# adjo0043/Mathematical-Modeling-Of-Infectious-Diseases-V1

Measured on AMD Instinct MI355X. Metric: ODE-solve+likelihood evals/sec (SEPAIHRD 4-age, 400d), higher is better.
Workload: dtype f64

## Files before the change

mathematical-modeling-of-infectious-diseases-v1_amd/csrc/phase_pass.py:

```python
#!/usr/bin/env python3
import argparse, os, re, subprocess, sys, tempfile

LLVM = "/opt/rocm/lib/llvm/bin"
MCPU = "gfx950"
E64_OK = re.compile(r"^\s+(v_fmac_f64_e32|v_mov_b32_e32|v_mov_b64_e32|v_add_u32_e32|v_sub_u32_e32|v_subrev_u32_e32|v_mul_f32_e32|v_add_f32_e32|"
                    r"v_cvt_f32_f64_e32|v_cvt_f64_f32_e32|v_cvt_f64_i32_e32|v_rcp_f64_e32|v_log_f32_e32|v_exp_f32_e32|v_and_b32_e32|v_or_b32_e32|"
                    r"v_lshlrev_b32_e32|v_max_i32_e32|v_min_i32_e32)\b")


def assemble_sizes(path):
    tmp = tempfile.mkdtemp(prefix="pp_")
    obj = os.path.join(tmp, "a.o")
    subprocess.run([LLVM + "/clang", "-x", "assembler", "-target", "amdgcn-amd-amdhsa", "-mcpu=" + MCPU, "-c", path, "-o", obj], check=True,
                   stdout=subprocess.DEVNULL, stderr=subprocess.DEVNULL)
    dis = subprocess.run([LLVM + "/llvm-objdump", "-d", obj], check=True, capture_output=True, text=True).stdout
    out, cur = {}, None
    for line in dis.splitlines():
        m = re.match(r"^[0-9a-f]+ <(\S+)>:", line)
        if m:
            cur = out.setdefault(m.group(1), [])
            continue
        m = re.match(r"^\s+(\S+).*//\s*([0-9A-Fa-f]+):\s+((?:[0-9A-Fa-f]{8}\s*)+)", line)
        if m and cur is not None:
            cur.append((int(m.group(2), 16), 4 * len(m.group(3).split()), m.group(1)))
# ... 72 lines not shown
        m = re.match(r"^(\w+):\s*(;.*)?$", l)
        if m and m.group(1) in sizes:
            func = m.group(1); funcs[func] = []
            continue
        if l.startswith("\t.end_amdhsa_kernel") or l.strip().startswith(".Lfunc_end"):
            func = None
        if func is not None and is_instruction(l):
            funcs[func].append(i)
    n_re = n_nop = n_runs = n_fixed = 0
    edits = {}
    inserts = {}
    for name, idxs in funcs.items():
        if not any(w in name for w in wanted):
            continue
        ins = sizes[name]
        if len(ins) != len(idxs):
            print(f"skip {name[:70]}: {len(ins)} disassembled vs {len(idxs)} listed instructions", file=sys.stderr)
            continue
        guarded = protected_spans(lines, idxs)
        start = 0
        shift = 0
        for k in range(len(ins) + 1):
            end_block = k == len(ins) or ins[k][2].startswith(("s_cbranch", "s_branch", "s_endpgm", "s_setpc"))
            if not end_block:
                continue
            blk = list(range(start, min(k + 1, len(ins))))
            start = k + 1
            if len(blk) < args.min_block:
                continue
            j = 0
            last_touch = -1
            while j < len(blk):
                a = blk[j]
                if ins[a][1] != 8:
                    j += 1
                    continue
                r = j
                while r < len(blk) and ins[blk[r]][1] == 8:
                    r += 1
                run_len = r - j
                if run_len >= args.min_run:
                    n_runs += 1
                    if (ins[a][0] + shift) % 8 == 4:
                        fixed = False
                        for b in range(j - 1, max(j - 1 - args.look_back, last_touch), -1):
                            li = idxs[blk[b]]
                            if blk[b] in guarded:
                                continue
                            if ins[blk[b]][1] == 4 and li not in edits and E64_OK.match(lines[li]) and "0x" not in lines[li] and "dpp" not in lines[li] and "sdwa" not in lines[li]:
                                edits[li] = lines[li].replace("_e32", "_e64", 1)
                                shift += 4; n_re += 1; fixed = True; last_touch = b
                                break
                        if not fixed and run_len >= args.nop_run and a not in guarded:
                            inserts[idxs[a]] = "\ts_nop 0"
                            shift += 4; n_nop += 1; fixed = True; last_touch = j
                        n_fixed += fixed
                j = r
    out = []
    for i, l in enumerate(lines):
        if i in inserts:
            out.append(inserts[i])
        out.append(edits.get(i, l))
    open(args.dst, "w").write("\n".join(out))
    try:
        after = assemble_sizes(args.dst)
    except subprocess.CalledProcessError:
        print("phase_pass: the rewritten assembly does not assemble", file=sys.stderr)
        sys.exit(1)
    if args.body_residue >= 0:
        out_lines = open(args.dst).read().split("\n")
        inserts_at = {}
        for name, ins in after.items():
            if "sepaihrd_eval_quad_kernel" not in name or not ins:
                continue
            blocks, start = [], 0
            for k in range(len(ins) + 1):
                if k == len(ins) or ins[k][2].startswith(("s_cbranch", "s_branch", "s_endpgm", "s_setpc")):
                    blocks.append(ins[start:min(k + 1, len(ins))]); start = k + 1
            bodies = [b for b in blocks if len(b) >= args.min_block and sum(1 for _, _, m in b if "f64" in m or "dpp" in m) * 2 > len(b)]
            if not bodies:
                continue
            body = min(bodies, key=len)
            delta = (args.body_residue - body[0][0]) % 64
            delta -= delta % 8
            if delta:
                inserts_at[name] = delta // 4
        if inserts_at:
            padded = []
            for l in out_lines:
                padded.append(l)
                m = re.match(r"^(\w+):\s*(;.*)?$", l)
                if m and m.group(1) in inserts_at:
                    padded.extend(["\ts_nop 0"] * inserts_at[m.group(1)])
            open(args.dst, "w").write("\n".join(padded))
            try:
                after = assemble_sizes(args.dst)
            except subprocess.CalledProcessError:
                print("phase_pass: the padded assembly does not assemble", file=sys.stderr)
                sys.exit(1)
            print(f"body residue {args.body_residue}: entry pads {sorted(set(inserts_at.values()))} s_nop in {len(inserts_at)} kernels")
    runs_before, off_before = off_phase_runs(sizes, wanted, args.min_run, args.min_block)
    runs_after, off_after = off_phase_runs(after, wanted, args.min_run, args.min_block)
    print(f"runs of >= {args.min_run} wide encodings: {n_runs}; off phase and fixed: {n_fixed} ({n_re} re-encoded, {n_nop} s_nop); "
          f"off-phase runs by the assembled addresses: {off_before} of {runs_before} before, {off_after} of {runs_after} after")
    if off_after > off_before:
        print("phase_pass: the rewritten assembly has MORE off-phase runs than its input", file=sys.stderr)
        sys.exit(1)


if __name__ == "__main__":
    main()
```

mathematical-modeling-of-infectious-diseases-v1_amd/csrc/sepaihrd_capi.cpp:

```cpp
#include "sepaihrd_hip.h"

#include <hip/hip_runtime.h>
#include <dlfcn.h>

#include <algorithm>
#include <cmath>
#include <cstdio>
#include <cstdlib>
#include <cstring>
#include <limits>
#include <string>
#include <vector>

#include "sepaihrd_device.h"
#include "sepaihrd_fd_device.h"
#include "sepaihrd_host_util.h"
#include "sepaihrd_mh_backend.h"
#include "sepaihrd_predictive_device.h"
#include "sepaihrd_segments.h"
#include "sepaihrd_stoch_sepaihrd_device.h"

using namespace sepaihrd;

enum EnsSlot {
// ... 263 lines not shown
    ctx->precision = pb->precision;
    ctx->n = n; ctx->T = T; ctx->P = P;
    ctx->host_N.assign(pb->N, pb->N + n);
    if (const char* mb = std::getenv("SEPAIHRD_WORKSPACE_MB")) {
        const long v = std::atol(mb);
        if (v > 0) ctx->ws_budget_bytes = (size_t)v << 20;
    }

    const int lpc = lanes_per_chain(n);
    const int ns = SS_SCHEDULE0 + nb + nk;

    std::vector<int32_t> src_scalar(ns, -1);
    std::vector<double> base_scalar(ns, 0.0);
    base_scalar[SS_BETA] = pb->beta; base_scalar[SS_THETA] = pb->theta; base_scalar[SS_SIGMA] = pb->sigma;
    base_scalar[SS_GAMMA_P] = pb->gamma_p; base_scalar[SS_GAMMA_A] = pb->gamma_A;
    base_scalar[SS_GAMMA_I] = pb->gamma_I; base_scalar[SS_GAMMA_H] = pb->gamma_H;
    base_scalar[SS_GAMMA_ICU] = pb->gamma_ICU;
    for (int i = 0; i < 8; ++i) base_scalar[SS_E0_MULT + i] = pb->multipliers[i];
    base_scalar[SS_RUNUP_DAYS] = pb->runup_days; base_scalar[SS_SEED_EXPOSED] = pb->seed_exposed;
    for (int k = 0; k < nb; ++k) base_scalar[SS_SCHEDULE0 + k] = pb->beta_values[k];
    for (int k = 0; k < nk; ++k) base_scalar[SS_SCHEDULE0 + nb + k] = pb->kappa_values[k];

    std::vector<int32_t> src_vec((size_t)VF_COUNT * lpc, -1);
    std::vector<double> base_vec((size_t)VF_COUNT * lpc, 0.0);
    const double* vec_base_ptr[VF_COUNT] = {pb->a, pb->h_infec, pb->p, pb->h, pb->icu, pb->d_H, pb->d_ICU,
                                            pb->d_community};
    for (int f = 0; f < VF_COUNT; ++f)
        for (int i = 0; i < n; ++i) base_vec[(size_t)f * lpc + i] = vec_base_ptr[f] ? vec_base_ptr[f][i] : 0.0;

    int kappa_calibrated = 0;
    for (int p = 0; p < P; ++p) {
        const int f = pb->param_field[p], idx = pb->param_index[p];
        auto bad = [&](const char* what) {
            set_err(err, errlen, std::string("param ") + std::to_string(p) + ": " + what);
            delete ctx;
            return static_cast<sepaihrd_ctx*>(nullptr);
        };
        if (f == SEPAIHRD_F_NONE) continue;
        if (f >= SEPAIHRD_F_BETA && f <= SEPAIHRD_F_SEED_EXPOSED) {
            src_scalar[f] = p;
        } else if (f == SEPAIHRD_F_BETA_VALUE) {
            if (idx < 0 || idx >= nb) return bad("beta index out of range");
            src_scalar[SS_SCHEDULE0 + idx] = p;
        } else if (f == SEPAIHRD_F_KAPPA_VALUE) {
            if (idx < 1 || idx >= nk) return bad("kappa index out of range (index 0 is the fixed baseline)");
            src_scalar[SS_SCHEDULE0 + nb + idx] = p;
            kappa_calibrated = 1;
        } else if (f >= SEPAIHRD_F_A && f <= SEPAIHRD_F_D_COMMUNITY) {
            if (idx < 0 || idx >= n) return bad("age index out of range");
            src_vec[(size_t)(f - SEPAIHRD_F_A) * lpc + idx] = p;
        } else {
            return bad("unknown field code");
        }
    }

    std::vector<double> Npad(lpc, 0.0), fracpad(lpc, 0.0), Mrow((size_t)lpc * lpc, 0.0),
        init((size_t)NUM_COMP * lpc, 0.0);
    double total_pop = 0.0;
    for (int i = 0; i < n; ++i) { Npad[i] = pb->N[i]; total_pop += pb->N[i]; }
    if (total_pop > 0.0)
        for (int i = 0; i < n; ++i) fracpad[i] = pb->N[i] / total_pop;
    for (int i = 0; i < n; ++i)
        for (int j = 0; j < n; ++j) Mrow[(size_t)i * lpc + j] = pb->M[(size_t)j * n + i];
    for (int c = 0; c < NUM_COMP; ++c)
        for (int i = 0; i < n; ++i) init[(size_t)c * lpc + i] = pb->initial_state[(size_t)c * n + i];

    int runup_offset = 0;
    for (int i = 0; i < T; ++i)
        if (pb->times[i] >= 0.0) { runup_offset = i; break; }
    const int num_obs_points = T - runup_offset;
    const int n_obs = pb->n_obs;
    const double qnan = std::numeric_limits<double>::quiet_NaN();
    std::vector<double> grid((size_t)T * lpc * 4, qnan);
    const double* obs_ptr[3] = {pb->obs_H, pb->obs_ICU, pb->obs_D};
    for (int k = 0; k < T; ++k)
        for (int i = 0; i < lpc; ++i) {
            double* rec = &grid[((size_t)k * lpc + i) * 4];
            const int r = k - runup_offset;
            if (i < n && r >= 0 && r < n_obs)
                for (int s = 0; s < 3; ++s) rec[s] = obs_ptr[s][(size_t)r * n + i];
            rec[3] = pb->times[k + 1 < T ? k + 1 : T - 1];
        }

    std::vector<double> mends;
    for (int k = 0; k < nb; ++k) mends.push_back(pb->beta_end_times[k]);
    for (int k = 0; k < nk; ++k) mends.push_back(pb->kappa_end_times[k]);
    std::sort(mends.begin(), mends.end());
    mends.erase(std::unique(mends.begin(), mends.end()), mends.end());
    const int nm = (int)mends.size();
    std::vector<int32_t> seg_ib(nm + 1, 0), seg_ik(nm + 1, 0);
    for (int j = 0; j <= nm; ++j) {
        const double trep = j < nm ? mends[j] : std::numeric_limits<double>::infinity();
        int cb = 0, ckk = 0;
        for (int k = 0; k < nb; ++k) cb += (trep > pb->beta_end_times[k]) ? 1 : 0;
        for (int k = 0; k < nk; ++k) ckk += (trep > pb->kappa_end_times[k]) ? 1 : 0;
        seg_ib[j] = nb > 0 ? std::min(cb, nb - 1) : 0;
        seg_ik[j] = std::min(ckk, nk - 1);
    }
    if (nm & 1) mends.push_back(std::numeric_limits<double>::infinity());

    double max_gap = 0.0;
    for (int i = 1; i < T; ++i) max_gap = std::max(max_gap, pb->times[i] - pb->times[i - 1]);

    ctx->lower.assign(P, 0.0); ctx->upper.assign(P, 0.0); ctx->has_bounds.assign(P, 0);
    std::vector<int32_t> hb(P, 0);
    for (int p = 0; p < P; ++p) {
        const bool has = pb->has_bounds ? pb->has_bounds[p] != 0 : (pb->lower && pb->upper);
        ctx->has_bounds[p] = has ? 1 : 0;
        hb[p] = has ? 1 : 0;
        if (has) { ctx->lower[p] = pb->lower[p]; ctx->upper[p] = pb->upper[p]; }
    }

    DevProblem& d = ctx->dp;
    d.n = n; d.lpc = lpc; d.T = T; d.n_obs = n_obs; d.runup_offset = runup_offset; d.nb = nb; d.nk = nk;
    d.P = P; d.ns = ns;
    d.constraint_mode = pb->constraint_mode == SEPAIHRD_CONSTRAINT_REFLECT ? 1 : 0;
    d.kappa_calibrated = kappa_calibrated;
    d.max_attempts = pb->max_attempts > 0 ? pb->max_attempts : 1000000;
    d.obs_rows_match = (num_obs_points == n_obs) ? 1 : 0;
    d.abs_tol = pb->abs_err; d.rel_tol = pb->rel_err; d.dt_hint = pb->dt_hint; d.max_gap = max_gap;

    bool ok = true;
    d.times = upload(ctx->allocs, std::vector<double>(pb->times, pb->times + T), ok);
    d.grid = upload(ctx->allocs, grid, ok);
    d.lower = upload(ctx->allocs, ctx->lower, ok);
    d.upper = upload(ctx->allocs, ctx->upper, ok);
    d.has_bounds = upload(ctx->allocs, hb, ok);
    d.src_scalar = upload(ctx->allocs, src_scalar, ok);
    d.base_scalar = upload(ctx->allocs, base_scalar, ok);
    d.src_vec = upload(ctx->allocs, src_vec, ok);
    d.base_vec = upload(ctx->allocs, base_vec, ok);
    d.N = upload(ctx->allocs, Npad, ok);
    d.age_fraction = upload(ctx->allocs, fracpad, ok);
    d.Mrow = upload(ctx->allocs, Mrow, ok);
    d.init_state = upload(ctx->allocs, init, ok);
    d.beta_ends = upload(ctx->allocs, std::vector<double>(pb->beta_end_times, pb->beta_end_times + nb), ok);
    d.kappa_ends = upload(ctx->allocs, std::vector<double>(pb->kappa_end_times, pb->kappa_end_times + nk), ok);
    d.nm = nm; d.nm_pad = (int)mends.size();
    d.mends = upload(ctx->allocs, mends, ok);
    d.seg_ib = upload(ctx->allocs, seg_ib, ok);
    d.seg_ik = upload(ctx->allocs, seg_ik, ok);
    if (!ok) {
        set_err(err, errlen, "device allocation / upload failed");
        sepaihrd_destroy(ctx);
        return nullptr;
    }
    if (eval_lds_bytes(d) + LOG_TABLE_LDS_BYTES > 64 * 1024) {
        set_err(err, errlen, "n_params too large for the LDS staging buffer");
        sepaihrd_destroy(ctx);
        return nullptr;
    }
    return ctx;
}

void sepaihrd_destroy(sepaihrd_ctx* ctx) {
    if (!ctx) return;
    (void)hipSetDevice(ctx->device);
    delete ctx;
}

const char* sepaihrd_last_error(const sepaihrd_ctx* ctx) { return ctx ? ctx->last_error.c_str() : "ctx is NULL"; }

int sepaihrd_set_constraint_mode(sepaihrd_ctx* ctx, int mode) {
    if (!ctx || (mode != SEPAIHRD_CONSTRAINT_CLAMP && mode != SEPAIHRD_CONSTRAINT_REFLECT))
        return SEPAIHRD_E_INVALID_ARG;
    ctx->dp.constraint_mode = mode;
    return SEPAIHRD_OK;
}

int sepaihrd_set_arith(sepaihrd_ctx* ctx, int arith) {
    if (!ctx || (arith != SEPAIHRD_ARITH_STRICT && arith != SEPAIHRD_ARITH_FMA)) return SEPAIHRD_E_INVALID_ARG;
    ctx->arith = arith;
    return SEPAIHRD_OK;
}

int sepaihrd_set_precision(sepaihrd_ctx* ctx, int precision) {
    if (!ctx || (precision != SEPAIHRD_PRECISION_F64 && precision != SEPAIHRD_PRECISION_F32)) return SEPAIHRD_E_INVALID_ARG;
    if (precision == SEPAIHRD_PRECISION_F32 && ctx->dp.lpc < 4) {
        ctx->last_error = "the fp32-state arm is built for 3 to 16 age classes";
        return SEPAIHRD_E_UNSUPPORTED;
    }
    if (precision == SEPAIHRD_PRECISION_F32 && ctx->solver == SEPAIHRD_SOLVER_FEHLBERG78) {
        ctx->last_error = "the fp32-state arm is built for Dopri5 and Cash-Karp only";
        return SEPAIHRD_E_UNSUPPORTED;
    }
    ctx->precision = precision;
    return SEPAIHRD_OK;
}

int sepaihrd_reserve(sepaihrd_ctx* ctx, int max_B) {
    if (!ctx || max_B < 0) return SEPAIHRD_E_INVALID_ARG;
    HIP_TRY(hipSetDevice(ctx->device), ctx, return SEPAIHRD_E_HIP);
    return ensure_workspace(ctx, chunk_chains(ctx, (size_t)max_B));
}

int sepaihrd_eval_batch_device(sepaihrd_ctx* ctx, const double* d_theta, int B, double* d_loglik,
                               int32_t* d_status, int32_t* d_n_accept, int32_t* d_n_reject,
                               double* d_ll_parts, double* d_traj, void* stream) {
    if (!ctx) return SEPAIHRD_E_INVALID_ARG;
    if (B < 0 || (B > 0 && (!d_theta || !d_loglik))) {
        ctx->last_error = "eval_batch_device: NULL theta/loglik or negative B";
        return SEPAIHRD_E_INVALID_ARG;
    }
    if (B == 0) return SEPAIHRD_OK;
    const int needs = needs_workspace(ctx, B, 0);
    if (needs < 0) { ctx->last_error = "unsupported lanes-per-chain"; return SEPAIHRD_E_UNSUPPORTED; }
    const bool split = needs != 0;
// ... 1910 lines not shown
```

mathematical-modeling-of-infectious-diseases-v1_amd/csrc/sepaihrd_device.h:

```cpp
#pragma once
#include <stdint.h>

namespace sepaihrd {

constexpr int NUM_COMP = 11;
constexpr int NUM_POP_COMP = 9;
constexpr int WAVE = 64;

enum ScalarSlot {
    SS_BETA = 0, SS_THETA, SS_SIGMA, SS_GAMMA_P, SS_GAMMA_A, SS_GAMMA_I, SS_GAMMA_H, SS_GAMMA_ICU,
    SS_E0_MULT, SS_P0_MULT, SS_A0_MULT, SS_I0_MULT, SS_H0_MULT, SS_ICU0_MULT, SS_R0_MULT, SS_D0_MULT,
    SS_RUNUP_DAYS, SS_SEED_EXPOSED,
    SS_SCHEDULE0
};
enum VecField { VF_A = 0, VF_H_INFEC, VF_P, VF_H, VF_ICU, VF_D_H, VF_D_ICU, VF_D_COMM, VF_COUNT };

struct DevProblem {
    int32_t n, lpc, T, n_obs, runup_offset, nb, nk, P, ns;
    int32_t constraint_mode, kappa_calibrated, max_attempts, obs_rows_match;
    int32_t init_mode;
    int32_t form;
    double abs_tol, rel_tol, dt_hint, max_gap;
    const double* times;
    const double* grid;
    const double* lower;
    const double* upper;
    const int32_t* has_bounds;
    const int32_t* src_scalar;
    const double* base_scalar;
    const int32_t* src_vec;
    const double* base_vec;
    const double* N;
    const double* age_fraction;
    const double* Mrow;
    const double* init_state;
    const double* beta_ends;
    const double* kappa_ends;
    int32_t nm, nm_pad;
    const double* mends;
    const int32_t* seg_ib;
    const int32_t* seg_ik;
};

struct EvalOutputs {
    double* loglik;
    int32_t* status;
    int32_t* n_accept;
    int32_t* n_reject;
    double* ll_parts;
    double* traj;
    double* cum;
    double* rows;
    int32_t* wstatus;
    void* ev_after_integrator;
    int32_t force_split;
};
inline size_t workspace_cum_doubles(const DevProblem& pb, size_t chains) { return (size_t)pb.T * 3 * chains * pb.lpc; }
constexpr size_t CUM_ROW_DOUBLES = 3 * WAVE;
#if defined(__HIPCC__)
__host__ __device__
#endif
inline size_t cum_index(int T, size_t column, int day, int comp) {
    return ((column / WAVE) * (size_t)T + (size_t)day) * CUM_ROW_DOUBLES + (size_t)comp * WAVE + (column % WAVE);
}
inline size_t workspace_rows_doubles(const DevProblem& pb, size_t chains) { return (size_t)pb.T * 3 * chains; }

constexpr int LL_FORM_INLINE = 0, LL_FORM_SEPARATE_PASS = 1, LL_FORM_CONSUMER_WAVES = 2;
struct LaunchInfo {
    int vgprs, sgprs, lds_static, lds_dynamic, scratch, max_blocks_per_cu;
    int lanes_per_chain;
    int likelihood_form;
    const char* name;
};

int launch_eval_strict(const DevProblem& pb, int solver, const double* d_theta, int B,
                       const EvalOutputs& out, void* stream);
int launch_eval_fma(const DevProblem& pb, int solver, const double* d_theta, int B,
                    const EvalOutputs& out, void* stream);
int launch_eval_scenario_strict(const DevProblem& pb, int solver, const double* d_theta, int B, const EvalOutputs& out, void* stream,
                                const double* d_kappa_mult, int stride);
int launch_eval_scenario_fma(const DevProblem& pb, int solver, const double* d_theta, int B, const EvalOutputs& out, void* stream,
                             const double* d_kappa_mult, int stride);
int launch_needs_workspace_strict(const DevProblem& pb, int solver, int B, int force_split);
int launch_needs_workspace_fma(const DevProblem& pb, int solver, int B, int force_split);
int launch_eval_f32(const DevProblem& pb, int solver, const double* d_theta, int B, const EvalOutputs& out, void* stream);
int kernel_info_f32(const DevProblem& pb, int solver, LaunchInfo* info);
int kernel_info_strict(const DevProblem& pb, int solver, int batch, LaunchInfo* info);
int kernel_info_fma(const DevProblem& pb, int solver, int batch, LaunchInfo* info);
int phase_pass_applied_strict();
int phase_pass_applied_fma();
int poisson_log_values(const double* d_x, int n, double* d_out, void* stream);

constexpr int ENSEMBLE_MAX_SAMPLES = 16384;
struct EnsembleArgs {
    int S, S_pad;
    int lpc, n, T, Tp;
    int runup_offset;
    int n_probs;
    size_t cum_stride;
    const double* cum;
    const int32_t* wstatus;
    const double* traj;
    double total_pop;
    double* vals;
    const double* probs;
    double* q_out;
    double* sero_out;
    int32_t* n_valid;
    double* rt_out;
    int rt_segment0;
    const DevProblem* pb;
    const double* theta;
    double* metrics_out;
    double* sort_scratch;
    size_t sort_scratch_doubles;
};
int launch_ensemble_summaries(const EnsembleArgs& a, void* stream);
struct ScenarioArgs {
    int K, S, S_pad, W;
    int n_probs;
    const double* probs;
    const double* metrics;
    const int32_t* wstatus;
    size_t status_stride;
    double* vals;
// ... 103 lines not shown
```

mathematical-modeling-of-infectious-diseases-v1_amd/csrc/sepaihrd_lane_split.inc:

```

constexpr int QUAD_LANES = 16;
constexpr int QUAD_CPW = WAVE / QUAD_LANES;
constexpr int QUAD_SLOTS = 3;

template <int CTRL>
__device__ __forceinline__ double quad_rot(double v) { return dpp_move<CTRL>(v); }
constexpr int QROT_LEFT = 0x93;
constexpr int QROT_NEXT = 0x39;

#ifndef SEPAIHRD_STRICT_STAGE_PADS
#define SEPAIHRD_STRICT_STAGE_PADS 0
#endif
#define SEP_STAGE_PAD(i, v) do { if ((SEPAIHRD_STRICT_STAGE_PADS >> (i)) & 1) asm volatile("s_nop 0" : "+v"(v)); } while (0)
#ifndef SEPAIHRD_STRICT_HEAD_PADS_CK
#define SEPAIHRD_STRICT_HEAD_PADS_CK 0
#endif
#ifndef SEPAIHRD_STRICT_STAGE_PADS_CK
#define SEPAIHRD_STRICT_STAGE_PADS_CK 0
#endif
#define SEP_STAGE_PAD_CK(i, v) do { if ((SEPAIHRD_STRICT_STAGE_PADS_CK >> (i)) & 1) asm volatile("s_nop 0" : "+v"(v)); } while (0)
#define SEP_PHASE_PAD(n) do { if ((n) >= 1) asm volatile("s_nop 0"); if ((n) >= 2) asm volatile("s_nop 0"); if ((n) >= 3) asm volatile("s_nop 0"); } while (0)
using lanemask = unsigned long long;
__device__ __forceinline__ lanemask lanes_where(bool p) { return __builtin_amdgcn_ballot_w64(p); }
__device__ __forceinline__ bool lane_of(lanemask m) { return __builtin_amdgcn_inverse_ballot_w64(m); }
__device__ __forceinline__ double min_plain(double a, double b) {
    double r;
    asm("v_min_f64 %0, %1, %2" : "=v"(r) : "v"(a), "v"(b));
    return r;
}

#if SEPAIHRD_ARITH_FMA
struct QuadModel {
    double theta_inf, m[4];
    double cO1, cL1;
    double cO0, cX0, cL0;
    double a1, a2, a3, a4, a5;
};

__device__ __forceinline__ void rhs_quad(const QuadModel& q, const double (&x)[QUAD_SLOTS], double (&dx)[QUAD_SLOTS],
                                         double beta_eff) {
    const double Lx1 = quad_rot<QROT_LEFT>(x[1]);
    const double Nx1 = quad_rot<QROT_NEXT>(x[1]), Nx0 = quad_rot<QROT_NEXT>(x[0]);
    const double pressure = fma(q.theta_inf, x[1], Lx1 + x[0]);
    double lambda = 0.0;
    fmac_row_bcast<2, 0xf, true>(lambda, pressure, q.m[0]);
    fmac_row_bcast<6, 0xf, false>(lambda, pressure, q.m[1]);
    fmac_row_bcast<10, 0xf, false>(lambda, pressure, q.m[2]);
    fmac_row_bcast<14, 0xf, false>(lambda, pressure, q.m[3]);
    lambda *= beta_eff;
    const double lambda_val = (0.0 < lambda) ? lambda : 0.0;
    const double W = lambda_val * x[0];
    dx[1] = fma(q.cO1, x[1], fma(q.cL1, Lx1, W));
    dx[0] = fma(q.cO0, x[0], fma(q.cX0, x[1], fma(q.cL0, Lx1, -W)));
    dx[2] = fma(q.a5, Nx0, fma(q.a4, x[0], fma(q.a3, Lx1, fma(q.a2, Nx1, q.a1 * x[1]))));
}

#else
struct QuadModel {
    double theta_inf, h_infec, inv_N, a_i, m[4];
    double u2, u3, v1, v2, v3;
    double u5, u6, u7, w1;
    double q1, q2, q3, q4, q5, q6;
};

__device__ __forceinline__ void rhs_quad(const QuadModel& q, const double (&x)[QUAD_SLOTS], double (&dx)[QUAD_SLOTS],
                                         double beta_eff) {
    const double Lx1 = quad_rot<QROT_LEFT>(x[1]);
    const double Nx1 = quad_rot<QROT_NEXT>(x[1]), Nx0 = quad_rot<QROT_NEXT>(x[0]);
    const double total_inf = Lx1 + x[0] + q.theta_inf * x[1];
    const double pressure = total_inf * q.h_infec * q.inv_N;
    double lambda = q.m[0] * dpp_bcast_row<2, 0xf, 2, 0x0>(pressure);
    lambda += q.m[1] * dpp_bcast_row<6, 0xf, 6, 0x0>(pressure);
    lambda += q.m[2] * dpp_bcast_row<10, 0xf, 10, 0x0>(pressure);
    lambda += q.m[3] * dpp_bcast_row<14, 0xf, 14, 0x0>(pressure);
    lambda *= beta_eff * q.a_i;
    const double lambda_val = (0.0 < lambda) ? lambda : 0.0;
    const double W = lambda_val * x[0];
    {
        const double t = q.u2 * Lx1;
        const double flow_in = (W + t) - q.u3 * t;
        const double out = q.v1 * x[1] + q.v2 * x[1] + q.v3 * x[1];
        dx[1] = flow_in - out;
    }
    {
        const double t5 = q.u5 * Lx1;
        const double flow_in = q.u6 * t5 + q.u7 * x[1];
        dx[0] = (flow_in - q.w1 * x[0]) - W;
    }
    dx[2] = q.q1 * x[0] + q.q2 * x[1] + q.q3 * Nx1 + q.q4 * Nx0 + q.q5 * x[0] + q.q6 * Lx1;
}

#endif

__device__ __forceinline__ int quad_comp(int cg, int slot) {
    if (slot == 0) return cg == 0 ? 0 : (cg == 1 ? -1 : (cg == 2 ? 3 : 6));
    if (slot == 1) return cg == 0 ? 1 : (cg == 1 ? 2 : (cg == 2 ? 4 : 5));
    return cg == 0 ? 10 : (cg == 1 ? 9 : (cg == 2 ? 7 : 8));
}

constexpr int QUAD_RING = 32;
constexpr int QUAD_BURST = 12;
constexpr int QUAD_UNITS = 4;
constexpr int QUAD_ROW_DOUBLES = QUAD_CPW * 12;
constexpr int QUAD_SPIN_LIMIT = 1 << 22;
constexpr size_t QUAD_FUSED_MAX_LDS = 144 * 1024;
constexpr int QUAD_CTRL_INTS = 8 + QUAD_UNITS * (2 * QUAD_CPW + 1 + 3 * QUAD_CPW);
constexpr int SEPAIHRD_STATUS_PIPELINE = 4;

SEP_HOST_DEVICE inline size_t quad_unit_doubles(const DevProblem& pb) {
    return (size_t)LDS_REC_DOUBLES + (size_t)QUAD_CPW * (pb.nm + 1) + (size_t)QUAD_CPW * pb.P + (size_t)QUAD_RING * QUAD_ROW_DOUBLES;
}
inline size_t quad_fused_lds_bytes(const DevProblem& pb) {
    const size_t need = ((size_t)times_pad(pb) + pb.nm_pad + QUAD_UNITS * quad_unit_doubles(pb)) * sizeof(double) + QUAD_CTRL_INTS * sizeof(int);
    constexpr size_t ONE_WORKGROUP_PER_CU = 82 * 1024;
    return need < ONE_WORKGROUP_PER_CU ? ONE_WORKGROUP_PER_CU : need;
}

struct QuadCtrl {
    int* produced;
    int* consumed;
    int* done;
    int* final_;
};
__device__ __forceinline__ QuadCtrl quad_ctrl(int* base, int unit) {
    int* u = base + 8 + unit * (2 * QUAD_CPW + 1 + 3 * QUAD_CPW);
    return QuadCtrl{u, u + QUAD_CPW, u + 2 * QUAD_CPW, u + 2 * QUAD_CPW + 1};
}
__device__ __forceinline__ int ld_acquire(const int* p) { return __hip_atomic_load(p, __ATOMIC_ACQUIRE, __HIP_MEMORY_SCOPE_WORKGROUP); }
__device__ __forceinline__ void st_release(int* p, int v) { __hip_atomic_store(p, v, __ATOMIC_RELEASE, __HIP_MEMORY_SCOPE_WORKGROUP); }

__device__ __forceinline__ void quad_ll_consumer(const DevProblem& pb, const EvalOutputs& out, const long long chain0, const int B,
                                              const double* ring, const QuadCtrl ctl) {
    const int lane = threadIdx.x & (WAVE - 1);
    const int c = lane >> 4, stream = (lane >> 2) & 3, age = lane & 3;
    const int s_ = stream < 3 ? stream : 0;
    const int src = (s_ == 0) ? 1 : (s_ == 1) ? 2 : 0;
    const bool chain_valid = chain0 + c < B;
    const double* cell = ring + c * 12 + src * 4 + age;
    const double* rec = pb.grid + (size_t)age * 4 + s_;
    double acc = 0.0;
    int k = 0, spins = 0;
    bool finished = false;
    const double* obs_k = rec;
    while (true) {
        const int fin = ld_acquire(ctl.done);
        const int avail = ld_acquire(ctl.produced + c);
        const bool burst = (avail - k >= QUAD_BURST) || fin != 0;
        if (__ballot(!finished && burst && k < avail) != 0ull) {
            int todo = finished ? 0 : avail - k;
            while (__ballot(todo > 0) != 0ull) {
                if (todo > 0) {
                    if (k >= pb.runup_offset) {
                        double inc = cell[(k & (QUAD_RING - 1)) * QUAD_ROW_DOUBLES];
                        inc = (inc < 0.0) ? 0.0 : inc;
                        const double obs = *obs_k;
                        const double sim = inc + 1e-10;
                        const double v = obs * log_pos(sim) - sim;
                        const double tv = (obs >= 0.0 && isfinite(obs)) ? v : 0.0;
                        double r = group_bcast<4, 0>(tv);
                        r += group_bcast<4, 1>(tv);
                        r += group_bcast<4, 2>(tv);
                        r += group_bcast<4, 3>(tv);
                        acc += r;
                    } else {
                        acc += 0.0;
                    }
                    ++k;
                    obs_k += 16;
                    --todo;
                }
            }
            if (!finished && stream == 0 && age == 0) st_release(ctl.consumed + c, k);
            spins = 0;
        } else {
            if (fin != 0) {
                if (!finished && k >= ld_acquire(ctl.produced + c)) finished = true;
            }
            if (__ballot(!finished) == 0ull) break;
            if (fin == 0) __builtin_amdgcn_s_sleep(96);
            if (++spins > QUAD_SPIN_LIMIT) break;
        }
    }
    const double h = dpp_bcast_row<0, 0xf, 0, 0x0>(acc), i = dpp_bcast_row<4, 0xf, 4, 0x0>(acc), d = dpp_bcast_row<8, 0xf, 8, 0x0>(acc);
    if (chain_valid && (lane & 15) == 0) {
        const long long chain = chain0 + c;
        int status = ctl.final_[3 * c + 0];
        if (spins > QUAD_SPIN_LIMIT && status == 0) status = SEPAIHRD_STATUS_PIPELINE;
        double total = (h + i) + d;
        const bool integ_ok = status == 0;
        if (status == 0 && (isnan(total) || isinf(total))) status = 1;
        if (status != 0) total = -DBL_MAX;
        out.loglik[chain] = total;
        if (out.status) out.status[chain] = status;
        if (out.n_accept) out.n_accept[chain] = ctl.final_[3 * c + 1];
        if (out.n_reject) out.n_reject[chain] = ctl.final_[3 * c + 2];
#ifndef SEPAIHRD_STAMPS
        if (out.ll_parts) {
            out.ll_parts[3 * chain + 0] = integ_ok ? h : 0.0;
            out.ll_parts[3 * chain + 1] = integ_ok ? i : 0.0;
            out.ll_parts[3 * chain + 2] = integ_ok ? d : 0.0;
        }
#endif
    }
}

#if !SEPAIHRD_ARITH_FMA
enum StrictCoefDopri5 { SD_B21 = 0, SD_B31, SD_B32, SD_B41, SD_B42, SD_B43, SD_B51, SD_B52, SD_B53, SD_B54, SD_B61, SD_B62, SD_B63, SD_B64,
                        SD_B65, SD_C1, SD_C3 , SD_C4, SD_C5, SD_C6, SD_DC1, SD_DC3, SD_DC4, SD_DC5, SD_DC6, SD_DC7 };
enum StrictCoefCashKarp { SK_A21 = 0, SK_A31, SK_A32, SK_A41, SK_A42, SK_A43, SK_A51, SK_A52, SK_A53, SK_A54, SK_A61, SK_A62, SK_A63, SK_A64,
                          SK_A65, SK_B1, SK_B3 , SK_B4, SK_B6, SK_DB1, SK_DB3, SK_DB4, SK_DB5, SK_DB6 };
__device__ const double STRICT_QUAD_COEF[2][2][16] = {
    {{dp::b21, dp::b31, dp::b32, dp::b41, dp::b42, dp::b43, dp::b51, dp::b52, dp::b53, dp::b54, dp::b61, dp::b62, dp::b63, dp::b64, dp::b65,
      dp::c1},
     {dp::c3, dp::c4, dp::c5, dp::c6, dp::dc1, dp::dc3, dp::dc4, dp::dc5, dp::dc6, dp::dc7, 0, 0, 0, 0, 0, 0}},
    {{ck::a21, ck::a31, ck::a32, ck::a41, ck::a42, ck::a43, ck::a51, ck::a52, ck::a53, ck::a54, ck::a61, ck::a62, ck::a63, ck::a64, ck::a65,
      ck::b1},
     {ck::b3, ck::b4, ck::b6, ck::db1, ck::db3, ck::db4, ck::db5, ck::db6, 0, 0, 0, 0, 0, 0, 0, 0}}};
template <int IDX>
__device__ __forceinline__ double strict_coef(double sA, double sB) {
    if constexpr (IDX < 16) return dpp_bcast_row<IDX, 0xf, IDX, 0x0>(sA);
    else return dpp_bcast_row<IDX - 16, 0xf, IDX - 16, 0x0>(sB);
}
#endif

template <int SOLVER, int ARITH, bool FUSED, bool TRAJ = true>
__global__ __launch_bounds__(FUSED ? 8 * WAVE : WAVE, 2) void sepaihrd_eval_quad_kernel(const DevProblem pb, const double* __restrict__ theta,
                                                                      const int B, const EvalOutputs out,
                                                                      const int cum_chains) {
    constexpr int LPC = 4, NS = QUAD_SLOTS, CPW = QUAD_CPW;
    extern __shared__ __attribute__((aligned(16))) double lds[];
    const int lane = threadIdx.x & (WAVE - 1);
    int unit = 0;
    double* unit_base;
    double* lds_times;
    double* lds_mends;
    int* ctrl_words = nullptr;
    if constexpr (FUSED) {
        lds_times = lds;
        lds_mends = lds + times_pad(pb);
        double* units0 = lds_mends + pb.nm_pad;
        ctrl_words = reinterpret_cast<int*>(units0 + QUAD_UNITS * quad_unit_doubles(pb));
        const int wave = threadIdx.x / WAVE;
        const int simd = (int)__builtin_amdgcn_s_getreg((1 << 11) | (4 << 6) | 4);
        if (lane == 0) ctrl_words[wave] = simd;
        for (int k = threadIdx.x; k < QUAD_CTRL_INTS - 8; k += 8 * WAVE) ctrl_words[8 + k] = 0;
        for (int k = threadIdx.x; k < pb.nm_pad; k += 8 * WAVE) lds_mends[k] = pb.mends[k];
        for (int k = threadIdx.x; k < pb.T; k += 8 * WAVE) lds_times[k] = pb.times[k];
        stage_log_table(threadIdx.x, 8 * WAVE);
        __syncthreads();
        int rank = 0, per_simd[4] = {0, 0, 0, 0};
        for (int w = 0; w < 8; ++w) {
            const int sw = ctrl_words[w] & 3;
            per_simd[sw]++;
            if (w < wave && sw == simd) ++rank;
        }
// ... 105 lines not shown
        q.u6 = (cg == 2) ? p : 0.0;
        q.u7 = (cg == 3) ? icu : 0.0;
        q.w1 = (cg == 2) ? gamma_A : (cg == 3 ? gamma_ICU + d_ICU : 0.0);
        q.q1 = (cg == 2) ? gamma_A : 0.0;
        q.q2 = (cg == 2) ? gamma_I : (cg == 3 ? d_H : 0.0);
        q.q3 = (cg == 1) ? h : (cg == 2 ? gamma_H : 0.0);
        q.q4 = (cg == 2) ? gamma_ICU : 0.0;
        q.q5 = (cg == 3) ? d_ICU : 0.0;
        q.q6 = (cg == 0) ? icu : (cg == 3 ? d_comm : 0.0);
#endif
    }

    Schedule sch;
    sch.me = lds_mends;
    {
        double* bkv = lds_bk + grp * (pb.nm + 1);
        for (int j = lane % QUAD_LANES; j <= pb.nm; j += QUAD_LANES) {
            const double beta = (pb.nb > 0) ? scalar_slot(SS_SCHEDULE0 + pb.seg_ib[j]) : scalar_slot(SS_BETA);
            const double kappa = scenario_kappa(pb, chain, pb.seg_ik[j], scalar_slot(SS_SCHEDULE0 + pb.nb + pb.seg_ik[j]));
            bkv[j] = beta * kappa;
        }
        sch.bkv = bkv;
    }

    int status = 0;
    if (pb.kappa_calibrated) {
        bool neg = false;
        for (int k = 1; k < pb.nk; ++k) neg |= (scalar_slot(SS_SCHEDULE0 + pb.nb + k) < 0.0);
        if (neg) status = 1;
    }
    if (!pb.obs_rows_match && pb.init_mode == 0) status = 1;

    double x[NS];
    SEP_UNROLL
    for (int s = 0; s < NS; ++s) {
        const int c = quad_comp(cg, s);
        x[s] = (c >= 0) ? pb.init_state[c * LPC + age] : 0.0;
    }
    if (pb.init_mode != 1) {
        const double runup_days = scalar_slot(SS_RUNUP_DAYS);
        const double seed_exposed = scalar_slot(SS_SEED_EXPOSED);
        const bool seeded = (pb.init_mode == 0 && runup_days > 0 && seed_exposed > 0);
        SEP_UNROLL
        for (int s = 0; s < NS; ++s) {
            const int c = quad_comp(cg, s);
            if (seeded) {
                if (c == 1) x[s] = seed_exposed * pb.age_fraction[age];
                else if (c >= 2) x[s] = 0.0;
            } else if (c >= 1 && c <= 8) {
                x[s] *= scalar_slot(SS_E0_MULT + (c - 1));
            }
        }
        double* cell = lds_scratch + (grp * LPC + age) * NUM_COMP;
        SEP_UNROLL
        for (int s = 0; s < NS; ++s) {
            const int c = quad_comp(cg, s);
            if (c >= 0) cell[c] = x[s];
        }
        wave_sync();
        double sum = 0;
        for (int c = 1; c < NUM_POP_COMP; ++c) sum += cell[c];
        if (group_any<QUAD_LANES>(sum > Ni || (pb.init_mode == 2 && sum < 0), lane)) status = 1;
        if (cg == 0) x[0] = Ni - sum;
    }
    wave_sync();

    int n_acc = 0, n_rej = 0;
    const int T = pb.T;

    const int which = (cg == 3) ? 0 : (cg == 1 ? 1 : 2);
    double* const cum_lane = FUSED ? nullptr : out.cum + cum_index(pb.T, (size_t)(chain0 + grp) * LPC + age, 0, which);
    const bool stores = chain_valid && cg != 2;
    auto obs_value = [&]() -> double { return x[2]; };
    double prev = obs_value();
    const int n_real = pb.n;
    double* cum_row = cum_lane;
    const size_t cum_step = CUM_ROW_DOUBLES;
    lanemask act = lanes_where(status == 0);
    int cons_seen = 0;
    int* const my_produced = FUSED ? ctl.produced + grp : nullptr;
    const int* const my_consumed = FUSED ? ctl.consumed + grp : nullptr;
    double* const ring_cell = lds_ring + grp * 12 + which * 4 + age;
    const bool ring_writer = cg != 2;
    int ring_budget = 0;
    auto observe_store = [&](lanemask do_m, int k) {
        if constexpr (FUSED) {
            if (__builtin_expect(ring_budget <= 0, 0)) {
                int spins = 0;
                do {
                    cons_seen = ld_acquire(my_consumed);
                    if ((do_m & lanes_where(k >= cons_seen + QUAD_RING)) == 0ull) break;
                    __builtin_amdgcn_s_sleep(2);
                } while (++spins < QUAD_SPIN_LIMIT);
                const lanemask stuck = do_m & lanes_where(k >= cons_seen + QUAD_RING);
                if (stuck != 0ull) {
                    if (lane_of(stuck)) status = SEPAIHRD_STATUS_PIPELINE;
                    act &= ~stuck;
                    do_m &= ~stuck;
                }
                const int slack = lane_of(act) ? cons_seen + QUAD_RING - k : QUAD_RING;
                const int s0 = __builtin_amdgcn_readlane(slack, 0), s1 = __builtin_amdgcn_readlane(slack, 16),
                          s2 = __builtin_amdgcn_readlane(slack, 32), s3 = __builtin_amdgcn_readlane(slack, 48);
                ring_budget = __builtin_amdgcn_readfirstlane(min(min(s0, s1), min(s2, s3)));
            }
            --ring_budget;
        }
        if (lane_of(do_m)) {
            const double v = obs_value();
            if constexpr (FUSED) {
                if (ring_writer) ring_cell[(k & (QUAD_RING - 1)) * QUAD_ROW_DOUBLES] = v - prev;
                if (cg == 0 && age == 0) st_release(my_produced, k + 1);
            } else {
                if (stores) *cum_row = v - prev;
                cum_row += cum_step;
            }
            prev = v;
            if constexpr (TRAJ) {
            if (out.traj != nullptr && chain_valid && age < n_real) {
                double* tdst = out.traj + ((size_t)chain * pb.T + k) * (NUM_COMP * n_real) + age;
                SEP_UNROLL
                for (int s = 0; s < NS; ++s) {
                    const int c = quad_comp(cg, s);
                    if (c >= 0) tdst[c * n_real] = x[s];
                }
            }
            }
        }
    };

    int k_next = 1;
    double t = pb.times[0];
    double dt = pb.dt_hint;
    int fails = 0;
    int attempts = 0;
    double t_next = (T > 1) ? pb.times[1] : t;
    double t_after = (T > 2) ? pb.times[2] : t_next;
    observe_store(act, 0);
    if (T <= 1) act = 0ull;

    sch.lo = INFINITY; sch.hi = -INFINITY; sch.bk = 0.0;
    double k1[NS];
    if (SOLVER == 0) {
        int c0, c1;
        segment_index2(sch, pb.nm_pad, t, t, c0, c1);
        rhs_quad(q, x, k1, sch.bkv[c0]);
    }
    const double eps_abs = pb.abs_tol, eps_rel = pb.rel_tol;
#if SEPAIHRD_ARITH_FMA
    const double coefA = QUAD_COEF[SOLVER][0][lane & 15], coefB = QUAD_COEF[SOLVER][1][lane & 15];
#else
    const double coefA = STRICT_QUAD_COEF[SOLVER][0][lane & 15], coefB = STRICT_QUAD_COEF[SOLVER][1][lane & 15];
#endif

#ifdef SEPAIHRD_STAMPS
    unsigned long long st0 = 0, st1 = 0, st2 = 0, st3 = 0, st4 = 0;
    unsigned long long acc_head = 0, acc_body = 0, acc_err = 0, acc_tail = 0;
#endif
    auto attempt = [&](const double cur, const double vecA, const double vecB, const double (&bks)[7]) __attribute__((always_inline)) {
        const bool active = lane_of(act);
        (void)active;
        SEP_STAMP(st1);
        double k2[NS], k3[NS], k4[NS], k5[NS], k6[NS], k7[NS];
        double xnew[NS], xerr[NS];
#if SEPAIHRD_ARITH_FMA
        rk_stages_row_coef<SOLVER, NS>(cur, vecA, vecB, x, k1, k2, k3, k4, k5, k6, k7, xnew, xerr, bks,
                                       [&](const double (&xin)[NS], double (&kout)[NS], double bk) { rhs_quad(q, xin, kout, bk); });
#else
        double xt[NS];
        if (SOLVER == 0) {
            { const double f1 = strict_coef<SD_B21>(vecA, vecB);
              SEP_UNROLL for (int c = 0; c < NS; ++c) xt[c] = x[c] + f1 * k1[c];
              rhs_quad(q, xt, k2, bks[1]); }
            SEP_STAGE_PAD(0, k2[0]);
            { const double f1 = strict_coef<SD_B31>(vecA, vecB), f2 = strict_coef<SD_B32>(vecA, vecB);
              SEP_UNROLL for (int c = 0; c < NS; ++c) xt[c] = x[c] + f1 * k1[c] + f2 * k2[c];
              rhs_quad(q, xt, k3, bks[2]); }
            SEP_STAGE_PAD(1, k3[0]);
            { const double f1 = strict_coef<SD_B41>(vecA, vecB), f2 = strict_coef<SD_B42>(vecA, vecB), f3 = strict_coef<SD_B43>(vecA, vecB);
              SEP_UNROLL for (int c = 0; c < NS; ++c) xt[c] = x[c] + f1 * k1[c] + f2 * k2[c] + f3 * k3[c];
              rhs_quad(q, xt, k4, bks[3]); }
            SEP_STAGE_PAD(2, k4[0]);
            { const double f1 = strict_coef<SD_B51>(vecA, vecB), f2 = strict_coef<SD_B52>(vecA, vecB), f3 = strict_coef<SD_B53>(vecA, vecB), f4 = strict_coef<SD_B54>(vecA, vecB);
              SEP_UNROLL for (int c = 0; c < NS; ++c)
                  xt[c] = x[c] + f1 * k1[c] + f2 * k2[c] + f3 * k3[c] + f4 * k4[c];
              rhs_quad(q, xt, k5, bks[4]); }
            SEP_STAGE_PAD(3, k5[0]);
            { const double f1 = strict_coef<SD_B61>(vecA, vecB), f2 = strict_coef<SD_B62>(vecA, vecB), f3 = strict_coef<SD_B63>(vecA, vecB), f4 = strict_coef<SD_B64>(vecA, vecB),
                           f5 = strict_coef<SD_B65>(vecA, vecB);
              SEP_UNROLL for (int c = 0; c < NS; ++c)
                  xt[c] = x[c] + f1 * k1[c] + f2 * k2[c] + f3 * k3[c] + f4 * k4[c] + f5 * k5[c];
              rhs_quad(q, xt, k6, bks[5]); }
            SEP_STAGE_PAD(4, k6[0]);
            { const double f1 = strict_coef<SD_C1>(vecA, vecB), f3 = strict_coef<SD_C3>(vecA, vecB), f4 = strict_coef<SD_C4>(vecA, vecB), f5 = strict_coef<SD_C5>(vecA, vecB),
                           f6 = strict_coef<SD_C6>(vecA, vecB);
              SEP_UNROLL for (int c = 0; c < NS; ++c)
                  xnew[c] = x[c] + f1 * k1[c] + f3 * k3[c] + f4 * k4[c] + f5 * k5[c] + f6 * k6[c];
              rhs_quad(q, xnew, k7, bks[6]); }
            SEP_STAGE_PAD(5, k7[0]);
            { const double e1 = strict_coef<SD_DC1>(vecA, vecB), e3 = strict_coef<SD_DC3>(vecA, vecB), e4 = strict_coef<SD_DC4>(vecA, vecB), e5 = strict_coef<SD_DC5>(vecA, vecB),
                           e6 = strict_coef<SD_DC6>(vecA, vecB), e7 = strict_coef<SD_DC7>(vecA, vecB);
              SEP_UNROLL for (int c = 0; c < NS; ++c)
                  xerr[c] = e1 * k1[c] + e3 * k3[c] + e4 * k4[c] + e5 * k5[c] + e6 * k6[c] + e7 * k7[c]; }
        } else {
            rhs_quad(q, x, k1, bks[0]);
            SEP_STAGE_PAD_CK(0, k1[0]);
            { const double f1 = strict_coef<SK_A21>(vecA, vecB);
              SEP_UNROLL for (int c = 0; c < NS; ++c) xt[c] = x[c] + f1 * k1[c];
// ... 266 lines not shown
```

Measured before the change: 8.456 million.

## Repack consumer likelihood loop by day with premasked observation records

The fused quad-kernel likelihood consumer now gives each lane a day instead of an age. It reads four ages per ring row with 16-byte LDS loads and uses a new host-built observation table with precomputed keep masks, so the per-element finite/nonnegative checks become bitmasks. Run-up rows are skipped by starting the consumed counter at the runup offset, and burst sizes are rounded to multiples of four days. Trajectory stores get their row base and offsets hoisted out of the step loop. The assembly phase pass also changes how it rounds the entry padding, which shifts code alignment.

```diff
diff --git a/mathematical-modeling-of-infectious-diseases-v1_amd/csrc/phase_pass.py b/mathematical-modeling-of-infectious-diseases-v1_amd/csrc/phase_pass.py
--- a/mathematical-modeling-of-infectious-diseases-v1_amd/csrc/phase_pass.py
+++ b/mathematical-modeling-of-infectious-diseases-v1_amd/csrc/phase_pass.py
@@ -178,7 +178,7 @@
                 continue
             body = min(bodies, key=len)
             delta = (args.body_residue - body[0][0]) % 64
-            delta -= delta % 8
+            delta = (delta + delta % 8) % 64
             if delta:
                 inserts_at[name] = delta // 4
         if inserts_at:
diff --git a/mathematical-modeling-of-infectious-diseases-v1_amd/csrc/sepaihrd_capi.cpp b/mathematical-modeling-of-infectious-diseases-v1_amd/csrc/sepaihrd_capi.cpp
--- a/mathematical-modeling-of-infectious-diseases-v1_amd/csrc/sepaihrd_capi.cpp
+++ b/mathematical-modeling-of-infectious-diseases-v1_amd/csrc/sepaihrd_capi.cpp
@@ -369,6 +369,23 @@
             rec[3] = pb->times[k + 1 < T ? k + 1 : T - 1];
         }
 
+    std::vector<double> cons_obs;
+    if (lpc == 4) {
+        const int rows = (num_obs_points > 0 ? (num_obs_points + 3) / 4 * 4 : 0) + 4;
+        cons_obs.assign((size_t)rows * 3 * CONS_REC_DOUBLES, 0.0);
+        for (int r = 0; r < num_obs_points; ++r)
+            for (int s = 0; s < 3; ++s) {
+                double* rec = &cons_obs[((size_t)r * 3 + s) * CONS_REC_DOUBLES];
+                uint32_t keep[4];
+                for (int i = 0; i < 4; ++i) {
+                    const double o = grid[((size_t)(runup_offset + r) * lpc + i) * 4 + s];
+                    rec[i] = o;
+                    keep[i] = (o >= 0.0 && std::isfinite(o)) ? 0xffffffffu : 0u;
+                }
+                std::memcpy(rec + 4, keep, sizeof keep);
+            }
+    }
+
     std::vector<double> mends;
     for (int k = 0; k < nb; ++k) mends.push_back(pb->beta_end_times[k]);
     for (int k = 0; k < nk; ++k) mends.push_back(pb->kappa_end_times[k]);
@@ -410,6 +427,7 @@
     bool ok = true;
     d.times = upload(ctx->allocs, std::vector<double>(pb->times, pb->times + T), ok);
     d.grid = upload(ctx->allocs, grid, ok);
+    d.cons_obs = cons_obs.empty() ? nullptr : upload(ctx->allocs, cons_obs, ok);
     d.lower = upload(ctx->allocs, ctx->lower, ok);
     d.upper = upload(ctx->allocs, ctx->upper, ok);
     d.has_bounds = upload(ctx->allocs, hb, ok);
diff --git a/mathematical-modeling-of-infectious-diseases-v1_amd/csrc/sepaihrd_device.h b/mathematical-modeling-of-infectious-diseases-v1_amd/csrc/sepaihrd_device.h
--- a/mathematical-modeling-of-infectious-diseases-v1_amd/csrc/sepaihrd_device.h
+++ b/mathematical-modeling-of-infectious-diseases-v1_amd/csrc/sepaihrd_device.h
@@ -40,7 +40,9 @@
     const double* mends;
     const int32_t* seg_ib;
     const int32_t* seg_ik;
-};
+    const double* cons_obs;
+};
+constexpr int CONS_REC_DOUBLES = 6;
 
 struct EvalOutputs {
     double* loglik;
diff --git a/mathematical-modeling-of-infectious-diseases-v1_amd/csrc/sepaihrd_lane_split.inc b/mathematical-modeling-of-infectious-diseases-v1_amd/csrc/sepaihrd_lane_split.inc
--- a/mathematical-modeling-of-infectious-diseases-v1_amd/csrc/sepaihrd_lane_split.inc
+++ b/mathematical-modeling-of-infectious-diseases-v1_amd/csrc/sepaihrd_lane_split.inc
@@ -103,6 +103,7 @@
 constexpr int QUAD_UNITS = 4;
 constexpr int QUAD_ROW_DOUBLES = QUAD_CPW * 12;
 constexpr int QUAD_SPIN_LIMIT = 1 << 22;
+static_assert(LDS_REC_DOUBLES % 2 == 0 && QUAD_CPW % 2 == 0 && QUAD_ROW_DOUBLES % 2 == 0, "the consumer reads a row's four ages with 16-byte LDS loads");
 constexpr size_t QUAD_FUSED_MAX_LDS = 144 * 1024;
 constexpr int QUAD_CTRL_INTS = 8 + QUAD_UNITS * (2 * QUAD_CPW + 1 + 3 * QUAD_CPW);
 constexpr int SEPAIHRD_STATUS_PIPELINE = 4;
@@ -129,48 +130,73 @@
 __device__ __forceinline__ int ld_acquire(const int* p) { return __hip_atomic_load(p, __ATOMIC_ACQUIRE, __HIP_MEMORY_SCOPE_WORKGROUP); }
 __device__ __forceinline__ void st_release(int* p, int v) { __hip_atomic_store(p, v, __ATOMIC_RELEASE, __HIP_MEMORY_SCOPE_WORKGROUP); }
 
+__device__ __forceinline__ double masked_term(double v, unsigned keep) {
+    return __hiloint2double((int)((unsigned)__double2hiint(v) & keep), (int)((unsigned)__double2loint(v) & keep));
+}
 __device__ __forceinline__ void quad_ll_consumer(const DevProblem& pb, const EvalOutputs& out, const long long chain0, const int B,
                                               const double* ring, const QuadCtrl ctl) {
     const int lane = threadIdx.x & (WAVE - 1);
-    const int c = lane >> 4, stream = (lane >> 2) & 3, age = lane & 3;
+    const int c = lane >> 4, stream = (lane >> 2) & 3, day = lane & 3;
     const int s_ = stream < 3 ? stream : 0;
     const int src = (s_ == 0) ? 1 : (s_ == 1) ? 2 : 0;
     const bool chain_valid = chain0 + c < B;
-    const double* cell = ring + c * 12 + src * 4 + age;
-    const double* rec = pb.grid + (size_t)age * 4 + s_;
+    const double* cell = ring + c * 12 + src * 4;
+    const int k0 = pb.runup_offset;
+    const double* rec0 = pb.cons_obs + ((size_t)day * 3 + s_) * CONS_REC_DOUBLES;
     double acc = 0.0;
-    int k = 0, spins = 0;
+    int k = k0, spins = 0;
     bool finished = false;
-    const double* obs_k = rec;
+    if (k0 > 0 && (lane & 15) == 0) st_release(ctl.consumed + c, k0);
     while (true) {
         const int fin = ld_acquire(ctl.done);
         const int avail = ld_acquire(ctl.produced + c);
-        const bool burst = (avail - k >= QUAD_BURST) || fin != 0;
-        if (__ballot(!finished && burst && k < avail) != 0ull) {
-            int todo = finished ? 0 : avail - k;
-            while (__ballot(todo > 0) != 0ull) {
-                if (todo > 0) {
-                    if (k >= pb.runup_offset) {
-                        double inc = cell[(k & (QUAD_RING - 1)) * QUAD_ROW_DOUBLES];
+        const int have = avail - k;
+        const bool burst = !finished && have > 0 && (have >= QUAD_BURST || fin != 0);
+        if (__ballot(burst) != 0ull) {
+            int take = finished ? 0 : (fin != 0 ? have : (have & ~3));
+            take = take > 0 ? take : 0;
+            const int k_end = k + take;
+            const int my_blocks = (take + 3) >> 2;
+            const int nb0 = __builtin_amdgcn_readlane(my_blocks, 0), nb1 = __builtin_amdgcn_readlane(my_blocks, 16),
+                      nb2 = __builtin_amdgcn_readlane(my_blocks, 32), nb3 = __builtin_amdgcn_readlane(my_blocks, 48);
+            const int blocks = __builtin_amdgcn_readfirstlane(max(max(nb0, nb1), max(nb2, nb3)));
+            int row = k + day;
+            const double* rec = rec0 + (size_t)(k - k0) * (3 * CONS_REC_DOUBLES);
+            for (int b = 0; b < blocks; ++b) {
+                if (b < my_blocks) {
+                    const double2* in2 = reinterpret_cast<const double2*>(cell + (row & (QUAD_RING - 1)) * QUAD_ROW_DOUBLES);
+                    const double2 i01 = in2[0], i23 = in2[1];
+                    const double in[4] = {i01.x, i01.y, i23.x, i23.y};
+                    const double2 o01 = *reinterpret_cast<const double2*>(rec), o23 = *reinterpret_cast<const double2*>(rec + 2);
+                    const uint4 keep = *reinterpret_cast<const uint4*>(rec + 4);
+                    const double obs[4] = {o01.x, o01.y, o23.x, o23.y};
+                    const unsigned kp[4] = {keep.x, keep.y, keep.z, keep.w};
+                    double sim[4], tv[4];
+                    LogLookup L[4];
+                    SEP_UNROLL
+                    for (int a = 0; a < 4; ++a) {
+                        double inc = in[a];
                         inc = (inc < 0.0) ? 0.0 : inc;
-                        const double obs = *obs_k;
-                        const double sim = inc + 1e-10;
-                        const double v = obs * log_pos(sim) - sim;
-                        const double tv = (obs >= 0.0 && isfinite(obs)) ? v : 0.0;
-                        double r = group_bcast<4, 0>(tv);
-                        r += group_bcast<4, 1>(tv);
-                        r += group_bcast<4, 2>(tv);
-                        r += group_bcast<4, 3>(tv);
-                        acc += r;
-                    } else {
-                        acc += 0.0;
+                        sim[a] = inc + 1e-10;
+                        L[a] = log_lookup(sim[a]);
                     }
-                    ++k;
-                    obs_k += 16;
-                    --todo;
+                    SEP_UNROLL
+                    for (int a = 0; a < 4; ++a) {
+                        const double v = obs[a] * log_finish(L[a]) - sim[a];
+                        tv[a] = masked_term(v, kp[a]);
+                    }
+                    double rs = ((tv[0] + tv[1]) + tv[2]) + tv[3];
+                    rs = (row < k_end) ? rs : 0.0;
+                    acc += group_bcast<4, 0>(rs);
+                    acc += group_bcast<4, 1>(rs);
+                    acc += group_bcast<4, 2>(rs);
+                    acc += group_bcast<4, 3>(rs);
+                    row += 4;
+                    rec += 4 * 3 * CONS_REC_DOUBLES;
                 }
             }
-            if (!finished && stream == 0 && age == 0) st_release(ctl.consumed + c, k);
+            k = k_end;
+            if (take > 0 && (lane & 15) == 0) st_release(ctl.consumed + c, k);
             spins = 0;
         } else {
             if (fin != 0) {
@@ -442,6 +468,20 @@
     const int* const my_consumed = FUSED ? ctl.consumed + grp : nullptr;
     double* const ring_cell = lds_ring + grp * 12 + which * 4 + age;
     const bool ring_writer = cg != 2;
+    double* traj_lane = nullptr;
+    int traj_row = 0, traj_off[NS] = {0, 0, 0};
+    bool traj_dup0 = false;
+    if constexpr (TRAJ) {
+        if (out.traj != nullptr && chain_valid && age < n_real) traj_lane = out.traj + (size_t)chain * pb.T * (NUM_COMP * n_real) + age;
+        traj_row = NUM_COMP * n_real;
+        SEP_UNROLL
+        for (int s = 0; s < NS; ++s) {
+            const int c = quad_comp(cg, s);
+            traj_off[s] = (c >= 0 ? c : quad_comp(cg, 1)) * n_real;
+        }
+        traj_dup0 = quad_comp(cg, 0) < 0;
+        asm volatile("" : "+v"(traj_lane), "+v"(traj_row), "+v"(traj_off[0]), "+v"(traj_off[1]), "+v"(traj_off[2]));
+    }
     int ring_budget = 0;
     auto observe_store = [&](lanemask do_m, int k) {
         if constexpr (FUSED) {
@@ -476,13 +516,11 @@
             }
             prev = v;
             if constexpr (TRAJ) {
-            if (out.traj != nullptr && chain_valid && age < n_real) {
-                double* tdst = out.traj + ((size_t)chain * pb.T + k) * (NUM_COMP * n_real) + age;
-                SEP_UNROLL
-                for (int s = 0; s < NS; ++s) {
-                    const int c = quad_comp(cg, s);
-                    if (c >= 0) tdst[c * n_real] = x[s];
-                }
+            if (traj_lane != nullptr) {
+                double* tdst = traj_lane + (size_t)k * traj_row;
+                tdst[traj_off[0]] = traj_dup0 ? x[1] : x[0];
+                tdst[traj_off[1]] = x[1];
+                tdst[traj_off[2]] = x[2];
             }
             }
         }
```

Result: no change. 8.520 million, median of 6 (+0.8%).
